# PetropoulakisPanagiotis/ICP-Variants

Measured on AMD Instinct MI355X. Metric: ICP iterations/s (k-NN + point-to-plane linear, 370k-point ETH-Apartment-like pair), higher is better.
Workload: dtype f32

## Files before the change

### icp-variants_amd/csrc/dev_fused.hpp

```cpp
struct RowSlotGen {
    const RowTerms& R;
    static constexpr int N = 27;
    template <int A> __device__ __forceinline__ double get() const { return row_slot<A>(R); }
};
struct P2pGen {
    float s[3], d[3]; double wd;
    static constexpr int N = 22;
    template <int A> __device__ __forceinline__ double get() const {
        double v;
        if constexpr (A < 3) v = (double)s[A];
        else if constexpr (A < 6) v = (double)d[A - 3];
        else if constexpr (A == 6) v = wd;
        else if constexpr (A < 10) v = wd * s[A - 7];
        else if constexpr (A < 13) v = wd * d[A - 10];
        else v = (double)d[(A - 13) / 3] * (wd * s[(A - 13) % 3]);
        return v;
    }
};
#ifndef ICP_FUSED_WAVES
#define ICP_FUSED_WAVES 6
#endif
#ifndef ICP_WAVE_STRIDE
#define ICP_WAVE_STRIDE (ICP_BVH_THREADS > 64 ? 128 : 0)
#endif
#ifndef ICP_DEBUG_WALK_ENDS
#define ICP_DEBUG_WALK_ENDS 0
#endif
#ifndef ICP_DEBUG_TIMES
#define ICP_DEBUG_TIMES 0
#endif
#if ICP_DEBUG_TIMES
#define ICP_STAMP(j) do { if (kp.dbg_steps && lane == 0) kp.dbg_steps[8 * (wave_slot) + (j)] = (int)(unsigned int)wall_clock64(); } while (0)
#define ICP_BUDGET_ROW(slot) ((kp.dbg_steps && 16 * kp.dbg_waves + 8 * 4096 <= kp.n) ? kp.dbg_steps + 8 * kp.dbg_waves + 8 * 4096 + 8 * (slot) : nullptr)
#else
#define ICP_STAMP(j)
#define ICP_BUDGET_ROW(slot) nullptr
#endif

template <int DIM> struct QueryIn {
    float r0, r1, r2;
    float c3, c4, c5;
    float rn0, rn1, rn2;
    int q0;
    float4 st;
    float4 ra, rb;
    float tq[DIM]; int j0;
};
template <int DIM>
__device__ __forceinline__ void fused_front_clear(QueryIn<DIM>& in) {
    in.r0 = 0.f; in.r1 = 0.f; in.r2 = 0.f; in.c3 = 0.f; in.c4 = 0.f; in.c5 = 0.f; in.rn0 = 0.f; in.rn1 = 0.f; in.rn2 = 0.f; in.q0 = -1; in.j0 = -1;
    in.st.x = 0.f; in.st.y = 0.f; in.st.z = 0.f; in.st.w = 0.f; in.ra = in.st; in.rb = in.st;
#pragma unroll
    for (int q = 0; q < DIM; q++) in.tq[q] = 0.f;
}
template <int DIM>
__device__ __forceinline__ void fused_front_loads(const KnnParams& kp, const PostParams& pp, const BvhViewT<DIM>& bv, int k, bool seeded, bool inc, QueryIn<DIM>& in) {
    fused_front_clear<DIM>(in);
    if (k >= 0) {
        const int i = kp.sel ? kp.sel[k] : k;
        in.r0 = kp.sx[i]; in.r1 = kp.sy[i]; in.r2 = kp.sz[i];
        if (DIM == 6) { in.c3 = kp.scr[i]; in.c4 = kp.scg[i]; in.c5 = kp.scb[i]; }
        in.rn0 = pp.snx[i]; in.rn1 = pp.sny[i]; in.rn2 = pp.snz[i];
        in.q0 = seeded ? kp.nn_raw[k] : -1;
        if (inc) in.st = kp.qstate[k];
        if (in.q0 >= 0) {
            if (DIM == 3) { in.ra = *(const float4*)(bv.recs + in.q0); in.rb = *((const float4*)(bv.recs + in.q0) + 1); in.tq[0] = in.ra.x; in.tq[1] = in.ra.y; in.tq[2] = in.ra.z; in.j0 = __float_as_int(in.ra.w); }
            else {
                const BvhLeafT<DIM>* lf = bv.leaves + (in.q0 >> 3);
#pragma unroll
                for (int q = 0; q < DIM; q++) in.tq[q] = lf->c[q][in.q0 & 7];
                in.j0 = lf->idx[in.q0 & 7];
            }
        }
    }
}

__host__ __device__ __forceinline__ int fused_wave_slot(int lb, int w, int mgrid) {
    constexpr int NW = BVH_THREADS / WAVE, S = ICP_WAVE_STRIDE;
    if (S == 0 || NW == 1) return lb * NW + w;
    if (S == 1) return w * mgrid + lb;
    const int g = lb / S, j = lb - g * S;
    return (g + 1) * S <= mgrid ? (g * NW + w) * S + j : lb * NW + w;
}

struct PairOut { bool valid; float s0, s1, s2, d0, d1, d2, n0, n1, n2, wt; };

template <int DIM, bool WIDE, bool XW = false>
__device__ __forceinline__ void fused_search_post(const KnnParams& kp, const BvhViewT<DIM>& bv, const PostParams& pp, int k, bool seeded, bool inc, const float* Pm, const float* Nm,
                                                  QueryIn<DIM>& in, uint2* __restrict__ bvh_lbq, int tid, int wave_slot, PairOut& o) {
    const int lane = tid & 63; (void)lane; (void)wave_slot; (void)seeded;
    o.valid = false; o.s0 = 0.f; o.s1 = 0.f; o.s2 = 0.f; o.d0 = 0.f; o.d1 = 0.f; o.d2 = 0.f; o.n0 = 0.f; o.n1 = 0.f; o.n2 = 0.f; o.wt = 0.f;
    float p[DIM];
#pragma unroll
    for (int q = 0; q < DIM; q++) p[q] = 0.f;
    if (DIM == 6) { p[3 % DIM] = in.c3; p[4 % DIM] = in.c4; p[5 % DIM] = in.c5; }
    float rn0 = in.rn0, rn1 = in.rn1, rn2 = in.rn2;
    float best = FLT_MAX, lb_others = 0.f; int bi = -1, bpos = -1, q0 = in.q0;
    float4 ra = in.ra, rb = in.rb;
#if ICP_DEBUG_TIMES
    float dbg_lbo = 0.f, dbg_lb3 = 0.f, dbg_delta = 0.f; int dbg_l2old = -1; const int dbg_q0old = in.q0;
#endif
    bool need_walk = false, verified = false, two_leaf = false;
    float lb3 = 0.f; int l2 = -1;
    if (k >= 0) {
        float2 st2; st2.x = 0.f; st2.y = __int_as_float(-1);
        xform_point(Pm, in.r0, in.r1, in.r2, p[0], p[1], p[2]);
        if (finite3(p[0], p[1], p[2]) && bv.n_valid > 0) {
            need_walk = true;
            if (q0 >= 0) {
                float d = 0.f;
#pragma unroll
                for (int q = 0; q < DIM; q++) { const float e = p[q] - in.tq[q]; d = (q == 0) ? e * e : d + e * e; }
                if (d < best) { best = d; bi = in.j0; bpos = q0; }
                if (inc && bi >= 0) {
                    const float ex = p[0] - in.st.x, ey = p[1] - in.st.y, ez = p[2] - in.st.z;
                    const float delta = sqrt_up((ex * ex + ey * ey) + ez * ez), sbest = sqrt_up(best);
                    const float lbn = (in.st.w - delta) * 0.999999f;
#if ICP_DEBUG_TIMES
                    dbg_lbo = in.st.w; dbg_lb3 = st2.x; dbg_delta = delta;
#endif
                    if (sbest < lbn) { lb_others = lbn; need_walk = false; verified = true; }
                    else {
                        if (kp.qstate2) st2 = kp.qstate2[k];
#if ICP_DEBUG_TIMES
                        dbg_l2old = __float_as_int(st2.y);
#endif
                        const float lb2 = (st2.x - delta) * 0.999999f;
                        l2 = __float_as_int(st2.y);
                        if (sbest < lb2) { two_leaf = true; lb3 = lb2; }
                    }
                }
            }
        }
    }
    ICP_STAMP(1);
#if ICP_DEBUG_TIMES
    if (kp.dbg_steps && k >= 0 && (need_walk || two_leaf) && seeded) {
        int* r = kp.dbg_steps + 8 * kp.dbg_waves + 8 * (k & 4095);
        r[0] = k; r[1] = __float_as_int(best); r[2] = __float_as_int(dbg_lbo); r[3] = __float_as_int(dbg_lb3); r[4] = __float_as_int(dbg_delta); r[5] = two_leaf ? l2 : -2; r[6] = q0; r[7] = (int)(unsigned int)wall_clock64();
    }
    if (kp.dbg_steps) { const int nw_ = __popcll(__ballot(need_walk && !two_leaf)), nl_ = __popcll(__ballot(two_leaf)); if (lane == 0) { kp.dbg_steps[8 * wave_slot + 6] = nw_ | (nl_ << 8);
            kp.dbg_steps[8 * wave_slot + 7] = (int)((__builtin_amdgcn_s_getreg((31 << 11) | 4) & 0xFFFFu) | (__builtin_amdgcn_s_getreg((31 << 11) | 20) << 16)); } }
#endif
    if (two_leaf) {
        f2 p2[DIM];
#pragma unroll
        for (int q = 0; q < DIM; q++) { p2[q].x = p[q]; p2[q].y = p[q]; }
        float b2 = FLT_MAX, b3 = FLT_MAX; int nl2 = -1;
        const int lf = q0 >> 3;
        if constexpr (DIM == 3) {
#pragma unroll 1
            for (int r = 0; r < 2; r++) {
                const int lx = r ? l2 : lf;
                if (r == 0 || (l2 >= 0 && l2 != lf)) leaf_eval<DIM>(bv.leaves + lx, lx, p2, best, bi, bpos, b2, nl2, b3);
            }
        } else {
            leaf_eval<DIM>(bv.leaves + lf, lf, p2, best, bi, bpos, b2, nl2, b3);
            if (l2 >= 0 && l2 != lf) leaf_eval<DIM>(bv.leaves + l2, l2, p2, best, bi, bpos, b2, nl2, b3);
        }
        lb_others = fminf(sqrt_dn(b2), lb3);
        lb3 = fminf(sqrt_dn(b3), lb3);
        l2 = nl2;
        need_walk = false;
    }
#if ICP_DEBUG_STEPS && !ICP_DEBUG_TIMES
    if (k >= 0 && kp.dbg_steps) kp.dbg_steps[k] = need_walk ? -1 : two_leaf ? -2 : 0;
#endif
#if ICP_DEBUG_TIMES
    if (int* row = ICP_BUDGET_ROW(wave_slot)) { if (lane < 8) row[lane] = 0; }
#endif
    bool walked = false;
    if (__any(need_walk)) {
        walked = true;
        float rn[3] = {rn0, rn1, rn2};
        knn_walk_shared<DIM, BVH_THREADS, typename std::conditional<WIDE, unsigned long long, unsigned int>::type, XW ? 1 : 0>(bv, p, rn, need_walk, best, bi, bpos, lb_others, lb3, l2, bvh_lbq, tid, kp.fault, ICP_BUDGET_ROW(wave_slot));
        rn0 = rn[0]; rn1 = rn[1]; rn2 = rn[2];
        q0 = -2;
        fused_front_clear<DIM>(in);
    }
    ICP_STAMP(2);
#if ICP_DEBUG_TIMES && ICP_DEBUG_WALK_ENDS
    if (k >= 0 && need_walk && seeded) {
        DEV_COUNT(8, 1);
        if (dbg_q0old >= 0 && (bpos >> 3) == (dbg_q0old >> 3)) DEV_COUNT(9, 1);
        if (dbg_l2old >= 0 && (bpos >> 3) == dbg_l2old) DEV_COUNT(10, 1);
    }
#endif
    asm volatile("" : "+v"(k));
    if (k >= 0) {
        if (!verified) knn_store_state<DIM>(kp, k, p, best, bpos, lb_others, lb3, l2);
        else if (kp.d2_out) kp.d2_out[k] = best;
        icp_match_t m;
        if (best <= kp.max_dist) { m.idx = bi; m.weight = 1.f; } else { m.idx = -1; m.weight = 0.f; }
        if (m.idx < 0) { if (pp.matches) pp.matches[k] = m; }
        else {
            if (walked || DIM != 3 || bpos != q0) { ra = *(const float4*)(bv.recs + bpos); rb = *((const float4*)(bv.recs + bpos) + 1); }
            o.d0 = ra.x; o.d1 = ra.y; o.d2 = ra.z; o.n0 = rb.x; o.n1 = rb.y; o.n2 = rb.z;
            o.s0 = p[0]; o.s1 = p[1]; o.s2 = p[2];
            o.valid = post_eval<true>(pp, k, m, o.d0, o.d1, o.d2, o.n0, o.n1, o.n2, __float_as_uint(rb.w), o.s0, o.s1, o.s2, o.wt, rn0, rn1, rn2, Nm);
        }
    }
    ICP_STAMP(3);
}

template <class StoreFn>
__device__ __forceinline__ void fused_block_epilogue(const KnnParams& kp, const PostParams& pp, PairOut& o, uint2* __restrict__ bvh_lbq, int tid, int wave_slot, const StoreFn& store) {
    constexpr int NW = BVH_THREADS / WAVE;
    const int lane = tid & 63, w = tid >> 6; (void)wave_slot; (void)kp;
    __syncthreads();
    double* lds = (double*)bvh_lbq;
    double tot;
    if (!o.valid) { o.s0 = 0.f; o.s1 = 0.f; o.s2 = 0.f; o.d0 = 0.f; o.d1 = 0.f; o.d2 = 0.f; o.n0 = 0.f; o.n1 = 0.f; o.n2 = 0.f; o.wt = 0.f; }
    if (pp.metric == ICP_METRIC_POINT_TO_PLANE) {
        RowTerms R;
        build_rows(0, o.s0, o.s1, o.s2, o.d0, o.d1, o.d2, o.n0, o.n1, o.n2, o.wt, R);
        const RowSlotGen g{R};
        tot = wave_transpose_reduce_gen<6, 0>(g, lane);
    } else {
        const P2pGen g{{o.s0, o.s1, o.s2}, {o.d0, o.d1, o.d2}, (double)o.wt};
        tot = wave_transpose_reduce_gen<6, 0>(g, lane);
    }
    ICP_STAMP(4);
    {
        const unsigned long long vm = __ballot(o.valid);
        const int v = wave_value_of_lane(lane);
        if (v < 32) lds[w * 32 + v] = tot;
        if (lane == 0) lds[NW * 32 + w] = (double)__popcll(vm);
    }
    __syncthreads();
    if (tid < NSUM_USED) {
        double out = 0.0;
        if (tid == SUM_N) { for (int ww = 0; ww < NW; ww++) out += lds[NW * 32 + ww]; }
        else {
            const int v = pp.metric == ICP_METRIC_POINT_TO_PLANE ? tid - SUM_M : tid - 1;
            const int nv = pp.metric == ICP_METRIC_POINT_TO_PLANE ? 27 : 22;
            if (v >= 0 && v < nv) { for (int ww = 0; ww < NW; ww++) out += lds[ww * 32 + v]; }
        }
        store(tid, out);
    }
    ICP_STAMP(5);
}

template <int DIM, bool WIDE, bool MERGED>
__device__ __forceinline__ void fused_matcher_body(const KnnParams& kp, const BvhViewT<DIM>& bv, const int* __restrict__ qorder, const PostParams& pp, const RingParams& rp) {
    extern __shared__ uint2 bvh_lbq[];
    constexpr int NW = BVH_THREADS / WAVE;
    if constexpr (MERGED) { if ((int)blockIdx.x < rp.n_red) { if (BVH_THREADS == RING_THREADS || threadIdx.x < RING_THREADS) ring_reduce_solve(rp); return; } }
    const int n_red = MERGED ? rp.n_red : 0;
    const int mblock = (int)blockIdx.x - n_red, mgrid = (int)gridDim.x - n_red;
    typedef const __attribute__((address_space(4))) float* cfloat_p;
    float Pm[16], Nm[9];
    if constexpr (!MERGED) {
        const cfloat_p pc = (cfloat_p)(const void*)kp.ps->pose; const cfloat_p nc = (cfloat_p)(const void*)kp.ps->nmat;
#pragma unroll
        for (int q = 0; q < 16; q++) Pm[q] = pc[q];
#pragma unroll
        for (int q = 0; q < 9; q++) Nm[q] = nc[q];
    }
    const int tid = threadIdx.x, lane = tid & 63, w = tid >> 6;
    if constexpr (MERGED) { if (rp.st.t0 && blockIdx.x == 0 && tid == 0) *rp.st.t0 = wall_clock64(); }
    const int lb = xcd_contiguous_block(mblock, mgrid);
    const int wave_slot = fused_wave_slot(lb, w, mgrid);
    const int t = wave_slot * BVH_QPW + lane;
    ICP_STAMP(0);
    const int k = ((BVH_QPW == WAVE || lane < BVH_QPW) && t < kp.n) ? (qorder ? qorder[t] : t) : -1;
    const bool seeded = kp.use_prev != 0, inc = kp.incremental && seeded;
    QueryIn<DIM> in;
    fused_front_loads<DIM>(kp, pp, bv, k, seeded, inc, in);
    constexpr bool XW = xw_enabled<DIM, BVH_THREADS>();
    if constexpr (XW) {
        xw_init<BVH_THREADS>(bvh_lbq, tid);
        asm volatile("s_waitcnt lgkmcnt(0)\n\ts_barrier" ::: "memory");
    }
    if constexpr (MERGED) { if (!ring_wait_pose(loop_slot((PoseState*)kp.ps, 0, (int)((blockIdx.x * 2u + (unsigned int)w) % (unsigned int)POSE_REPLICAS)), lane, rp.run_fault, Pm, Nm)) return; }
    PairOut o;
    fused_search_post<DIM, WIDE, XW>(kp, bv, pp, k, seeded, inc, Pm, Nm, in, bvh_lbq, tid, wave_slot, o);
    if constexpr (XW) {
        if (xw_block_is_searching<BVH_THREADS>(bvh_lbq)) {
            constexpr int NT = BVH_THREADS;
            bvh_lbq[3 * NT + tid] = make_uint2(__float_as_uint(o.s0), __float_as_uint(o.s1)); bvh_lbq[4 * NT + tid] = make_uint2(__float_as_uint(o.s2), __float_as_uint(o.d0));
            bvh_lbq[5 * NT + tid] = make_uint2(__float_as_uint(o.d1), __float_as_uint(o.d2)); bvh_lbq[7 * NT + tid] = make_uint2(__float_as_uint(o.n0), __float_as_uint(o.n1));
            bvh_lbq[8 * NT + tid] = make_uint2(__float_as_uint(o.n2), __float_as_uint(o.wt)); bvh_lbq[9 * NT + tid] = make_uint2(o.valid ? 1u : 0u, 0u);
            xw_help<DIM, NT, typename std::conditional<WIDE, unsigned long long, unsigned int>::type>(bv, bvh_lbq, tid, kp.fault, ICP_BUDGET_ROW(wave_slot));
            const uint2 a = bvh_lbq[3 * NT + tid], b = bvh_lbq[4 * NT + tid], c = bvh_lbq[5 * NT + tid], d = bvh_lbq[7 * NT + tid], e = bvh_lbq[8 * NT + tid], f = bvh_lbq[9 * NT + tid];
            o.s0 = __uint_as_float(a.x); o.s1 = __uint_as_float(a.y); o.s2 = __uint_as_float(b.x); o.d0 = __uint_as_float(b.y); o.d1 = __uint_as_float(c.x); o.d2 = __uint_as_float(c.y);
            o.n0 = __uint_as_float(d.x); o.n1 = __uint_as_float(d.y); o.n2 = __uint_as_float(e.x); o.wt = __uint_as_float(e.y); o.valid = f.x != 0u;
        }
    }
    double* partials = pp.partials;
    fused_block_epilogue(kp, pp, o, bvh_lbq, tid, wave_slot, [=](int a, double v) { partials[(size_t)a * mgrid + lb] = v; });
    if constexpr (MERGED) { if (rp.st.block_t1 && tid == 0) rp.st.block_t1[lb] = wall_clock64(); }
}
template <int DIM, bool WIDE>
__global__ __launch_bounds__(BVH_THREADS, DIM == 3 ? ICP_FUSED_WAVES : 4) void k_knn_bvh_post(const KnnParams kp, const BvhViewT<DIM> bv, const int* __restrict__ qorder, const PostParams pp) {
    const RingParams none{};
    fused_matcher_body<DIM, WIDE, false>(kp, bv, qorder, pp, none);
}
template <int DIM, bool WIDE>
__global__ __launch_bounds__(BVH_THREADS, DIM == 3 ? ICP_FUSED_WAVES : 4) void k_knn_bvh_post_ring(const KnnParams kp, const BvhViewT<DIM> bv, const int* __restrict__ qorder, const PostParams pp, const RingParams rp) {
    static_assert(BVH_THREADS >= RING_THREADS, "the reducer blocks are the first RING_THREADS threads of a matcher-sized block");
    fused_matcher_body<DIM, WIDE, true>(kp, bv, qorder, pp, rp);
}
```

### icp-variants_amd/csrc/dev_solve.hpp

```cpp
template <int n, int COPY>
__device__ inline void jacobi_eig_sym(double* A , double* V, double* ev) {
#pragma unroll
    for (int i = 0; i < n; i++) {
#pragma unroll
        for (int j = 0; j < n; j++) V[i * n + j] = (i == j) ? 1.0 : 0.0;
    }
    for (int sweep = 0; sweep < 50; sweep++) {
        double off = 0.0, dg = 0.0;
#pragma unroll
        for (int i = 0; i < n; i++) {
#pragma unroll
            for (int j = 0; j < n; j++) { if (i != j) off += A[i * n + j] * A[i * n + j]; else dg += A[i * n + j] * A[i * n + j]; }
        }
        if (off <= 1e-300 || off <= 1e-34 * dg) break;
#pragma unroll
        for (int p = 0; p < n - 1; p++) {
#pragma unroll
            for (int q = p + 1; q < n; q++) {
                const double apq = A[p * n + q];
                if (apq != 0.0) {
                    const double theta = (A[q * n + q] - A[p * n + p]) / (2.0 * apq);
                    const double t = (theta >= 0 ? 1.0 : -1.0) / (fabs(theta) + sqrt(theta * theta + 1.0));
                    const double c = 1.0 / sqrt(t * t + 1.0), s = t * c;
#pragma unroll
// ... 266 lines not shown
}
template <int COPY = 0>
__device__ __forceinline__ bool solve_p2plane_lanes(const SolveParams& sp, const double* tot ) {
    if (!(sp.update_pose && sp.metric == ICP_METRIC_POINT_TO_PLANE && sp.phase == 0 && tot[SUM_N] > 0)) return false;
    PoseState* ps = sp.ps;
    const float* npose = p2plane_lanes_core<COPY>(tot + SUM_M, ps->pose);
    if (!npose) return false;
    const int tid = threadIdx.x;
    if (tid == 0 && sp.sums_out) for (int a = 0; a < NSUM; a++) sp.sums_out[a] = tot[a];
    if (tid >= 64 && tid < 70) {
        const int k = tid - 64; const double n = tot[SUM_N];
        if (k < 3) ps->mean_s[k] = (float)(tot[SUM_S + k] / n); else ps->mean_d[k - 3] = (float)(tot[SUM_D + k - 3] / n);
    }
    if (tid < 16) { ps->pose[tid] = npose[tid]; if (sp.stats) sp.stats->pose[tid] = npose[tid]; }
    if (tid >= 32 && tid < 41) ps->nmat[tid - 32] = normal_matrix_entry(npose, tid - 32);
    if (tid == 33 && sp.stats) {
        sp.stats->n_src = sp.n_src; sp.stats->n_valid = (int)tot[SUM_N];
        sp.stats->rmse = -1.f; sp.stats->benchmark_error = -1.f; sp.stats->status = ICP_OK;
    }
    return true;
}

template <bool WITH_SYMMETRIC, int COPY = 0>
__device__ inline void solve_generic(const SolveParams& sp, const double* tot) {
    if (sp.sums_out) for (int a = 0; a < NSUM; a++) sp.sums_out[a] = tot[a];
    PoseState* ps = sp.ps;
    const double n = tot[SUM_N];
    if (sp.phase == 0) {
        float ms[3] = {0, 0, 0}, md[3] = {0, 0, 0};
        if (n > 0) for (int k = 0; k < 3; k++) { ms[k] = (float)(tot[SUM_S + k] / n); md[k] = (float)(tot[SUM_D + k] / n); }
        for (int k = 0; k < 3; k++) { ps->mean_s[k] = ms[k]; ps->mean_d[k] = md[k]; }
    }
    if (!sp.update_pose) return;
    if (sp.metric == ICP_METRIC_SYMMETRIC && sp.phase == 0) return;
    int status = ICP_OK;
    float dT[16];
    for (int i = 0; i < 16; i++) dT[i] = (i % 5 == 0) ? 1.f : 0.f;
    if (!(n > 0)) {
        status = ICP_ERR_NO_CORRESPONDENCES;
    } else if (sp.metric == ICP_METRIC_POINT_TO_PLANE) {
        double x[6];
        solve_normal_svd<COPY>(tot + SUM_M, x);
        const float al = (float)x[0], be = (float)x[1], ga = (float)x[2];
        const float ca = (float)cos((double)al), sa = (float)sin((double)al);
        const float cb = (float)cos((double)be), sb = (float)sin((double)be);
        const float cg = (float)cos((double)ga), sg = (float)sin((double)ga);
        const float Rx[9] = {1, 0, 0, 0, ca, -sa, 0, sa, ca}, Ry[9] = {cb, 0, sb, 0, 1, 0, -sb, 0, cb}, Rz[9] = {cg, -sg, 0, sg, cg, 0, 0, 0, 1};
        float Rxy[9], R[9];
        mat3_mul_f32(Rx, Ry, Rxy); mat3_mul_f32(Rxy, Rz, R);
        const float t[3] = {(float)x[3], (float)x[4], (float)x[5]};
        set_pose_f32(dT, R, t);
    } else if (sp.metric == ICP_METRIC_POINT_TO_POINT) {
        const double* m = tot + SUM_M;
        const float msf[3] = {ps->mean_s[0], ps->mean_s[1], ps->mean_s[2]}, mdf[3] = {ps->mean_d[0], ps->mean_d[1], ps->mean_d[2]};
        __shared__ double A[9], Rd[9];
        for (int j = 0; j < 3; j++) for (int k = 0; k < 3; k++)
            A[j * 3 + k] = m[7 + j * 3 + k] - m[4 + j] * (double)msf[k] - (double)mdf[j] * m[1 + k] + m[0] * (double)mdf[j] * (double)msf[k];
        double mom = 0.0;
        for (int i = 0; i < 9; i++) mom = fmax(mom, fabs(m[7 + i]));
        float R[9];
        procrustes_rotation<COPY>(A, (RANK_CUT3 * RANK_CUT3) * mom, Rd);
        for (int i = 0; i < 9; i++) R[i] = (float)Rd[i];
        const float tr[3] = {mdf[0] - msf[0], mdf[1] - msf[1], mdf[2] - msf[2]};
        float t[3];
        for (int r = 0; r < 3; r++) {
            const float Rt = R[r * 3] * tr[0] + (R[r * 3 + 1] * tr[1] + R[r * 3 + 2] * tr[2]);
            const float Rm = R[r * 3] * mdf[0] + (R[r * 3 + 1] * mdf[1] + R[r * 3 + 2] * mdf[2]);
            t[r] = (Rt - Rm) + mdf[r];
        }
        set_pose_f32(dT, R, t);
    } else if constexpr (WITH_SYMMETRIC) {
        __shared__ double M[36], g[6], x[6], ywork[6];
        __shared__ int colp[6];
        int q = 0;
        for (int a = 0; a < 6; a++) for (int c = a; c < 6; c++) { M[a * 6 + c] = tot[SUM_M + q]; M[c * 6 + a] = tot[SUM_M + q]; q++; }
        for (int a = 0; a < 6; a++) g[a] = tot[SUM_M + 21 + a];
        const float lambda = 0.0001f; const float l2 = lambda * lambda;
        for (int a = 0; a < 6; a++) M[a * 6 + a] += (double)l2;
        solve_fullpiv_lu6<COPY>(M, g, x, colp, ywork);
        const float at[3] = {(float)x[0], (float)x[1], (float)x[2]}, tt[3] = {(float)x[3], (float)x[4], (float)x[5]};
        const float tan_theta = sqrtf(at[0] * at[0] + (at[1] * at[1] + at[2] * at[2]));
        const float ax[3] = {at[0] / tan_theta, at[1] / tan_theta, at[2] / tan_theta};
        const float sin_theta = (float)((double)tan_theta / sqrt(1.0 + (double)(tan_theta * tan_theta)));
        const float cos_theta = sin_theta / tan_theta;
        const float t[3] = {tt[0] * cos_theta, tt[1] * cos_theta, tt[2] * cos_theta};
        const float K[9] = {0, -ax[2], ax[1], ax[2], 0, -ax[0], -ax[1], ax[0], 0};
        float Ks[9], KK[9], Rod[9];
        const float omc = 1 - cos_theta;
        for (int i = 0; i < 9; i++) Ks[i] = omc * K[i];
        mat3_mul_f32(Ks, K, KK);
        for (int i = 0; i < 9; i++) Rod[i] = ((i % 4 == 0) ? 1.f : 0.f) + (sin_theta * K[i] + KK[i]);
        const float I3[9] = {1, 0, 0, 0, 1, 0, 0, 0, 1}, zero[3] = {0, 0, 0};
        const float md[3] = {ps->mean_d[0], ps->mean_d[1], ps->mean_d[2]}, nms[3] = {-ps->mean_s[0], -ps->mean_s[1], -ps->mean_s[2]};
        float Tm[16], Tt[16], Ts[16], Rm[16], t1[16], t2[16];
        set_pose_f32(Tm, I3, md); set_pose_f32(Tt, I3, t); set_pose_f32(Ts, I3, nms); set_pose_f32(Rm, Rod, zero);
        mat4_mul_f32(Tm, Rm, t1); mat4_mul_f32(t1, Tt, t2); mat4_mul_f32(t2, Rm, t1); mat4_mul_f32(t1, Ts, dT);
    }
    if (status == ICP_OK) {
        float np[16];
        mat4_mul_f32(dT, ps->pose, np);
        for (int i = 0; i < 16; i++) ps->pose[i] = np[i];
        normal_matrix_from_pose(ps->pose, ps->nmat);
    }
    if (sp.stats) {
        sp.stats->n_src = sp.n_src;
        sp.stats->n_valid = (int)n;
        for (int i = 0; i < 16; i++) sp.stats->pose[i] = ps->pose[i];
        sp.stats->rmse = -1.f;
        sp.stats->benchmark_error = -1.f;
        sp.stats->status = status;
    }
}

template <bool WITH_SYMMETRIC = true, int COPY = 0>
__device__ __forceinline__ void solve_tail(const SolveParams& sp, const double* tot) {
    if (solve_p2plane_lanes<COPY>(sp, tot)) return;
    if (threadIdx.x == 0) solve_generic<WITH_SYMMETRIC, COPY>(sp, tot);
}

constexpr int SOLVE_THREADS = 256;
constexpr unsigned long long TOTAL_SENTINEL = 0xFFF8D1CEC0DE5EEDull;
constexpr int SPIN_LIMIT = 1 << 22;
constexpr int SOLVE_INFLIGHT = 12;
__global__ __launch_bounds__(SOLVE_THREADS) void k_reduce_solve(const SolveParams sp) {
#include "dev_body_reduce_solve.hpp"
}


#ifndef ICP_POSE_REPLICAS
#define ICP_POSE_REPLICAS 16
#endif
constexpr int POSE_REPLICAS = ICP_POSE_REPLICAS;
constexpr size_t POSE_REPLICA_STRIDE = 4096 + 128;
__device__ __host__ __forceinline__ PoseState* loop_slot(PoseState* base, int g, int replica) {
    return (PoseState*)((char*)base + ((size_t)g * POSE_REPLICAS + (size_t)replica) * POSE_REPLICA_STRIDE);
}
__global__ void k_run_init(const PoseState src, PoseState* ps_copy, PoseState* slots, int n_slots, unsigned long long* totals, int n_totals, int* zero_words, int n_zero,
                           unsigned long long* stamps, int n_stamps) {
    const int t = blockIdx.x * blockDim.x + threadIdx.x;
    const int n_slot_granules = n_slots * POSE_REPLICAS * 16;
    if (t < n_slot_granules) {
        const int g = t / (POSE_REPLICAS * 16), r = (t / 16) % POSE_REPLICAS, q = t & 15;
        unsigned long long* dst = (unsigned long long*)loop_slot(slots, g, r) + q;
        *dst = g == 0 ? ((const unsigned long long*)&src)[q] : ~0ull;
        if (g == 0 && r == 0 && ps_copy) ((unsigned long long*)ps_copy)[q] = ((const unsigned long long*)&src)[q];
    } else if (t < n_slot_granules + n_totals) totals[t - n_slot_granules] = ~0ull;
    else if (t < n_slot_granules + n_totals + n_zero) zero_words[t - n_slot_granules - n_totals] = 0;
    else if (t < n_slot_granules + n_totals + n_zero + n_stamps) stamps[t - n_slot_granules - n_totals - n_zero] = 0ull;
}
constexpr unsigned long long GRANULE_EMPTY = ~0ull;
#ifndef ICP_RING_SLEEP
#define ICP_RING_SLEEP 4
#endif
struct RingStamps {
    unsigned long long* t0; unsigned long long* block_t1;
    const unsigned long long* prev_block_t1; unsigned long long* prev_t1;
    unsigned long long* end;
};
struct RingParams {
    const double* red_partials; int red_nblocks;
    unsigned long long* totals_row;
    const PoseState* ps_in;
    PoseState* ps_out;
    icp_iter_stats* stats; int n_src;
    PoseState* final_out;
    int* words_out;
    int* run_fault;
    int n_red;
    ConvergeParams cv;
    RingStamps st;
};
__device__ __forceinline__ unsigned long long granule_of(unsigned int lo, unsigned int hi) {
    const unsigned long long g = ((unsigned long long)hi << 32) | lo;
    return g == GRANULE_EMPTY ? g ^ 1ull : g;
}
constexpr int RING_THREADS = 128;
#ifndef ICP_DEBUG_TIMES
#define ICP_DEBUG_TIMES 0
#endif
#if ICP_DEBUG_TIMES
__device__ int g_ring_dbg[(NSUM_USED + 1) * 8];
#define RING_STAMP(a, j) do { if (threadIdx.x == 0 && !rp.final_out) g_ring_dbg[8 * (a) + (j)] = (int)(unsigned int)wall_clock64(); } while (0)
#else
#define RING_STAMP(a, j)
#endif
__device__ __forceinline__ void ring_close(const RingParams& rp) {
    if (threadIdx.x != 0) return;
    if (rp.words_out) {
        int wds[16];
#pragma unroll
        for (int k = 0; k < 16; k++) wds[k] = __hip_atomic_load(rp.run_fault + k, __ATOMIC_RELAXED, __HIP_MEMORY_SCOPE_AGENT);
#pragma unroll
        for (int k = 0; k < 16; k++) rp.words_out[k] = wds[k];
    }
    if (rp.st.end) *rp.st.end = wall_clock64();
}
__device__ __forceinline__ void ring_reduce_solve(const RingParams& rp) {
    __shared__ double tot[NSUM];
    __shared__ double wsum[4];
    __shared__ unsigned int slot_words[32];
    __shared__ int give_up;
    const int tid = threadIdx.x, lane = tid & 63, w = tid >> 6, a = blockIdx.x;
    RING_STAMP(a, 0);
    if (a == 0 && tid == 0 && rp.st.t0) *rp.st.t0 = wall_clock64();
    if (a == 0 && rp.ps_in->fault) {
        { const unsigned int* src = (const unsigned int*)rp.ps_in; for (int q = tid; q < 16 * POSE_REPLICAS; q += RING_THREADS) __hip_atomic_store((unsigned long long*)loop_slot(rp.ps_out, 0, q >> 4) + (q & 15), granule_of(src[2 * (q & 15)], src[2 * (q & 15) + 1]), __ATOMIC_RELAXED, __HIP_MEMORY_SCOPE_AGENT);
          if (rp.final_out && tid < 32) ((unsigned int*)rp.final_out)[tid] = src[tid]; }
        ring_close(rp);
        return;
    }
    {
        const double* __restrict__ row = rp.red_partials + (size_t)a * rp.red_nblocks;
        double x0 = 0.0, x1 = 0.0;
        for (int b0 = 0; b0 < rp.red_nblocks; b0 += SOLVE_INFLIGHT * SOLVE_THREADS) {
            double v0[SOLVE_INFLIGHT], v1[SOLVE_INFLIGHT];
#pragma unroll
            for (int j = 0; j < SOLVE_INFLIGHT; j++) {
                const int b = b0 + j * SOLVE_THREADS + tid;
                v0[j] = b < rp.red_nblocks ? row[b] : 0.0;
                v1[j] = b + RING_THREADS < rp.red_nblocks ? row[b + RING_THREADS] : 0.0;
            }
#pragma unroll
            for (int j = 0; j < SOLVE_INFLIGHT; j++) {
                const int b = b0 + j * SOLVE_THREADS + tid;
                if (b < rp.red_nblocks) x0 += v0[j];
                if (b + RING_THREADS < rp.red_nblocks) x1 += v1[j];
            }
        }
        for (int off = 32; off > 0; off >>= 1) { x0 += __shfl_down(x0, off, WAVE); x1 += __shfl_down(x1, off, WAVE); }
        if (lane == 0) { wsum[w] = x0; wsum[2 + w] = x1; }
    }
    RING_STAMP(a, 1);
    __syncthreads();
    if (tid == 0) {
        double x = wsum[0];
        for (int k = 1; k < 4; k++) x += wsum[k];
        const unsigned long long bits = (unsigned long long)__double_as_longlong(x);
        __hip_atomic_store(rp.totals_row + a, granule_of((unsigned int)bits, (unsigned int)(bits >> 32)), __ATOMIC_RELAXED, __HIP_MEMORY_SCOPE_AGENT);
    }
    RING_STAMP(a, 2);
    if (a == 1 && rp.st.prev_t1) {
        static_assert(RING_THREADS == 2 * WAVE, "two wave maxima meet below");
        __shared__ unsigned long long tmax[RING_THREADS / WAVE];
        unsigned long long m = 0ull;
        for (int b = tid; b < rp.red_nblocks; b += RING_THREADS) { const unsigned long long v = rp.st.prev_block_t1[b]; m = v > m ? v : m; }
        for (int off = 32; off > 0; off >>= 1) { const unsigned long long v = __shfl_down(m, off, WAVE); m = v > m ? v : m; }
        if (lane == 0) tmax[w] = m;
        __syncthreads();
        if (tid == 0) *rp.st.prev_t1 = tmax[0] > tmax[1] ? tmax[0] : tmax[1];
    }
    if (a != 0) return;
    if (tid == 0) give_up = 0;
    __syncthreads();
    if (tid < NSUM) {
        double v = 0.0;
        if (tid < NSUM_USED) {
            unsigned long long bits = GRANULE_EMPTY;
            for (int spin = 0; spin < SPIN_LIMIT; spin++) {
                bits = __hip_atomic_load(rp.totals_row + tid, __ATOMIC_RELAXED, __HIP_MEMORY_SCOPE_AGENT);
                if (bits != GRANULE_EMPTY) break;
                __builtin_amdgcn_s_sleep(2);
            }
            if (bits == GRANULE_EMPTY) give_up = 1;
            v = __longlong_as_double((long long)bits);
        }
        tot[tid] = v;
    }
    __syncthreads();
    RING_STAMP(NSUM_USED, 0);
    const PoseState* pin = rp.ps_in;
    const double n = tot[SUM_N];
    int fault = 0, status = ICP_OK;
    const float* npose = nullptr;
    if (give_up) { fault = 1; if (tid == 0) atomicOr(rp.run_fault, 1); }
    else if (n > 0) { npose = p2plane_lanes_core(tot + SUM_M, pin->pose); if (!npose) fault = 2; }
    else status = ICP_ERR_NO_CORRESPONDENCES;
    RING_STAMP(NSUM_USED, 1);
    int code = fault;
    if (rp.cv.on && !fault) {
        if (tid < WAVE && converge_step(rp.cv, npose ? npose : pin->pose, pin->pose, status == ICP_OK, tid)) code = SLOT_STOPPED;
    }
    if (tid < 16) slot_words[tid] = __float_as_uint(npose ? npose[tid] : pin->pose[tid]);
    if (tid >= 32 && tid < 41) slot_words[16 + tid - 32] = __float_as_uint(npose ? normal_matrix_entry(npose, tid - 32) : pin->nmat[tid - 32]);
    if (tid >= 64 && tid < 70) {
        const int k = tid - 64;
        slot_words[25 + k] = __float_as_uint(n > 0 ? (float)(tot[(k < 3 ? SUM_S : SUM_D - 3) + k] / n) : 0.f);
    }
    if (tid == 0) slot_words[31] = (unsigned int)code;
    __syncthreads();
    for (int q = tid; q < 16 * POSE_REPLICAS; q += RING_THREADS)
        __hip_atomic_store((unsigned long long*)loop_slot(rp.ps_out, 0, q >> 4) + (q & 15), granule_of(slot_words[2 * (q & 15)], slot_words[2 * (q & 15) + 1]), __ATOMIC_RELAXED, __HIP_MEMORY_SCOPE_AGENT);
    RING_STAMP(NSUM_USED, 2);
    if (rp.final_out && tid < 32) ((unsigned int*)rp.final_out)[tid] = slot_words[tid];
    if (rp.stats && !fault) {
        if (tid < 16) rp.stats->pose[tid] = __uint_as_float(slot_words[tid]);
        if (tid == 16) { rp.stats->n_src = rp.n_src; rp.stats->n_valid = (int)n; rp.stats->rmse = -1.f; rp.stats->benchmark_error = -1.f; rp.stats->status = status; }
    }
    ring_close(rp);
}
__global__ __launch_bounds__(RING_THREADS) void k_ring_reduce_solve(const RingParams rp) { ring_reduce_solve(rp); }

__device__ __forceinline__ bool ring_wait_pose(const PoseState* slot, int lane, int* run_fault, float (&Pm)[16], float (&Nm)[9]) {
    const unsigned long long* g = (const unsigned long long*)slot;
    unsigned long long v = 0ull;
    bool ok = false;
    for (int spin = 0; spin < SPIN_LIMIT; spin++) {
        if (lane < 16) v = __hip_atomic_load(g + lane, __ATOMIC_RELAXED, __HIP_MEMORY_SCOPE_AGENT);
        if (!__any(lane < 16 && v == GRANULE_EMPTY)) { ok = true; break; }
        __builtin_amdgcn_s_sleep(ICP_RING_SLEEP);
    }
    if (!ok) { if (lane == 0) atomicOr(run_fault, 1); return false; }
    const int lo = (int)(unsigned int)v, hi = (int)(unsigned int)(v >> 32);
#pragma unroll
    for (int q = 0; q < 16; q++) Pm[q] = __int_as_float(__builtin_amdgcn_readlane((q & 1) ? hi : lo, q >> 1));
#pragma unroll
    for (int q = 0; q < 9; q++) Nm[q] = __int_as_float(__builtin_amdgcn_readlane(((16 + q) & 1) ? hi : lo, (16 + q) >> 1));
    return __builtin_amdgcn_readlane(hi, 15) == 0;
}
```

### icp-variants_amd/csrc/host_launch.hpp

```cpp
namespace {
struct MergeLaunch { RingParams rp; const PoseState* slot; double* partials; };

constexpr size_t WALK_LDS_BYTES = (size_t)ICP_SHARE_ROWS * BVH_THREADS * 8;
template <int DIM> size_t fused_lds_bytes() {
    const size_t red_bytes = (size_t)(BVH_THREADS / WAVE) * 33 * 8;
    return (WALK_LDS_BYTES > red_bytes ? WALK_LDS_BYTES : red_bytes) + xw_lds_bytes<DIM, BVH_THREADS>();
}
int post_nblocks(int n) { const int nb = (n + POST_THREADS - 1) / POST_THREADS; return nb > POST_BLOCKS ? POST_BLOCKS : nb < 1 ? 1 : nb; }
template <class K> K pick_wide(int Lq, K narrow, K wide) { return Lq <= 8 ? narrow : wide; }

struct QuerySet { const Cloud* cl; const int* sel; int n; int pretransformed; bool use_colors; bool seed_prev; const int* order; bool keep_records = false; };

int ensure_qpack(icp_ctx* c, int n) {
    if ((size_t)n <= c->q_cap && c->qpack.p) return ICP_OK;
    int rc;
    c->q_cap = ((size_t)n + 63) / 64 * 64;
    if ((rc = ensure(c, c->qpack, c->q_cap * 28))) return rc;
    set_view(c->nn_raw, c->qpack.p, c->q_cap * 4); set_view(c->qstate, c->qpack.as<char>() + c->q_cap * 4, c->q_cap * 16);
    set_view(c->qstate2, c->qpack.as<char>() + c->q_cap * 20, c->q_cap * 8);
    return ICP_OK;
}

KnnParams knn_params(const icp_ctx* c, const Cloud& q, const int* sel, int n) {
    KnnParams kp; memset(&kp, 0, sizeof(kp));
    kp.sx = q.x.as<float>(); kp.sy = q.y.as<float>(); kp.sz = q.z.as<float>(); kp.scr = q.cr.as<float>(); kp.scg = q.cg.as<float>(); kp.scb = q.cb.as<float>();
    kp.sel = sel; kp.n = n;
    kp.tx = c->tgt.x.as<float>(); kp.ty = c->tgt.y.as<float>(); kp.tz = c->tgt.z.as<float>();
    kp.tcr = c->tgt.cr.as<float>(); kp.tcg = c->tgt.cg.as<float>(); kp.tcb = c->tgt.cb.as<float>();
    kp.mpad = c->tgt.npad; kp.max_dist = c->prm.max_distance; kp.nseg = 1;
    return kp;
}

PostParams make_post_params(icp_ctx* c, const Cloud& src, const int* sel, int n) {
    const icp_params& p = c->prm;
    PostParams pp;
    pp.sx = src.x.as<float>(); pp.sy = src.y.as<float>(); pp.sz = src.z.as<float>();
    pp.snx = src.nx.as<float>(); pp.sny = src.ny.as<float>(); pp.snz = src.nz.as<float>();
    pp.srgba = src.rgba.as<uint32_t>(); pp.sel = sel; pp.n = n;
    pp.tx = c->tgt.x.as<float>(); pp.ty = c->tgt.y.as<float>(); pp.tz = c->tgt.z.as<float>();
    pp.tnx = c->tgt.nx.as<float>(); pp.tny = c->tgt.ny.as<float>(); pp.tnz = c->tgt.nz.as<float>(); pp.trgba = c->tgt.rgba.as<uint32_t>();
    pp.ps = c->ps.as<PoseState>(); pp.matches = c->matches.as<icp_match_t>();
    pp.metric = p.metric; pp.weighting = p.weighting; pp.rejection = p.rejection;
    pp.max_dist = p.max_distance; pp.cos_reject = c->cos_reject; pp.partials = c->partials.as<double>();
    return pp;
}

template <int DIM>
int launch_bvh_query(icp_ctx* c, Bvh& b, const CoordPtrs<DIM>& cp, const KnnParams& kp, const int* order, int n, const Cloud* fuse, bool keep_records, int* fused_blocks, const MergeLaunch* ml = nullptr) {
    int rc;
    if (!b.valid && (rc = build_bvh<DIM>(c, b, cp))) return rc;
    const BvhViewT<DIM> bv = make_view<DIM>(b, cp);
    const int nb = fuse ? fused_nblocks(n) : (n + BVH_THREADS - 1) / BVH_THREADS;
    if (fuse) {
        if ((rc = ensure(c, c->partials, (size_t)(nb > POST_BLOCKS ? nb : POST_BLOCKS) * NSUM * 8))) return rc;
        PostParams pp = make_post_params(c, *fuse, kp.sel, n);
        KnnParams kf = kp; kf.out = nullptr;
        if (!keep_records) { pp.matches = nullptr; kf.d2_out = nullptr; }
        const size_t lds = fused_lds_bytes<DIM>();
        if (ml) {
            kf.ps = ml->slot; pp.ps = ml->slot; pp.partials = ml->partials; kf.fault = ml->rp.run_fault;
            const auto ring = pick_wide(b.Lq, k_knn_bvh_post_ring<DIM, false>, k_knn_bvh_post_ring<DIM, true>);
            hipLaunchKernelGGL(ring, dim3(nb + ml->rp.n_red), dim3(BVH_THREADS), lds, c->stream, kf, bv, order, pp, ml->rp);
        }
        else hipLaunchKernelGGL(pick_wide(b.Lq, k_knn_bvh_post<DIM, false>, k_knn_bvh_post<DIM, true>), dim3(nb), dim3(BVH_THREADS), lds, c->stream, kf, bv, order, pp);
        *fused_blocks = nb;
    } else hipLaunchKernelGGL(k_knn_bvh<DIM>, dim3(nb), dim3(BVH_THREADS), WALK_LDS_BYTES, c->stream, kp, bv, order);
    HIPCK(c, hipGetLastError());
    return ICP_OK;
}

int launch_match(icp_ctx* c, const QuerySet& q, int* fused_blocks = nullptr, const MergeLaunch* ml = nullptr) {
    const icp_params& p = c->prm;
    int rc;
    if (fused_blocks) *fused_blocks = 0;
    if ((rc = ensure(c, c->matches, (size_t)q.n * sizeof(icp_match_t))) || (rc = ensure(c, c->d2, (size_t)q.n * 4))) return rc;
    if (p.matching == ICP_MATCH_PROJECTIVE) {
        ProjParams pp;
        pp.sx = q.cl->x.as<float>(); pp.sy = q.cl->y.as<float>(); pp.sz = q.cl->z.as<float>(); pp.sel = q.sel; pp.n = q.n;
        pp.tx = c->tgt.x.as<float>(); pp.ty = c->tgt.y.as<float>(); pp.tz = c->tgt.z.as<float>();
        pp.width = p.width; pp.height = p.height; pp.fx = p.fx; pp.fy = p.fy; pp.mx = p.cx; pp.my = p.cy; pp.window = 12;
        pp.ps = c->ps.as<PoseState>(); pp.pretransformed = q.pretransformed; pp.max_dist = p.max_distance;
        pp.out = c->matches.as<icp_match_t>(); pp.d2_out = c->d2.as<float>();
        hipLaunchKernelGGL(k_projective, dim3((q.n + 255) / 256), dim3(256), 0, c->stream, pp);
        HIPCK(c, hipGetLastError());
        return ICP_OK;
    }
    KnnParams kp = knn_params(c, *q.cl, q.sel, q.n);
    kp.ps = c->ps.as<PoseState>(); kp.pretransformed = q.pretransformed; kp.fault = &c->ps.as<PoseState>()->fault;
    kp.out = c->matches.as<icp_match_t>(); kp.d2_out = c->d2.as<float>();
    if (p.knn_backend == ICP_KNN_LBVH) {
        if ((rc = ensure_qpack(c, q.n))) return rc;
        kp.nn_raw = c->nn_raw.as<int>(); kp.use_prev = q.seed_prev ? 1 : 0;
#if ICP_DEBUG_STEPS
        if ((rc = ensure(c, c->dbg_steps, (size_t)q.n * 4))) return rc;
        kp.dbg_steps = c->dbg_steps.as<int>(); kp.dbg_waves = fused_nblocks(q.n) * (BVH_THREADS / WAVE);
#endif
        if (p.knn_incremental && !q.pretransformed) {
            kp.qstate = c->qstate.as<float4>(); kp.qstate2 = c->qstate2.as<float2>(); kp.incremental = 1;
        }
        const Cloud* fuse = (fused_blocks != nullptr && p.metric != ICP_METRIC_SYMMETRIC && p.metric != ICP_METRIC_GICP && p.metric != ICP_METRIC_COLORED && !q.pretransformed) ? q.cl : nullptr;
        if (q.use_colors) return launch_bvh_query<6>(c, c->bvh6, target_coords6(c), kp, q.order, q.n, fuse, q.keep_records, fused_blocks, fuse ? ml : nullptr);
        return launch_bvh_query<3>(c, c->bvh, target_coords3(c), kp, q.order, q.n, fuse, q.keep_records, fused_blocks, fuse ? ml : nullptr);
    }
    const int bx = (q.n + WAVE - 1) / WAVE;
    const int nch = kp.mpad / KNN_CH;
    int nseg = 1;
    if (bx < 1024) { nseg = (2048 + bx - 1) / bx; if (nseg > nch / 4) nseg = nch / 4; if (nseg < 1) nseg = 1; }
    kp.nseg = nseg;
    if (nseg > 1) {
        if ((rc = ensure(c, c->best64, (size_t)q.n * 8))) return rc;
        kp.best64 = c->best64.as<unsigned long long>();
        const unsigned long long init = ((unsigned long long)0x7F7FFFFFu << 32) | 0xFFFFFFFFull;
        hipLaunchKernelGGL(k_fill_u64, dim3((q.n + 255) / 256), dim3(256), 0, c->stream, kp.best64, q.n, init);
    }
    if (q.use_colors) hipLaunchKernelGGL(k_knn_brute<6>, dim3(bx, nseg), dim3(256), 0, c->stream, kp);
    else              hipLaunchKernelGGL(k_knn_brute<3>, dim3(bx, nseg), dim3(256), 0, c->stream, kp);
    if (nseg > 1)
        hipLaunchKernelGGL(k_knn_finalize, dim3((q.n + 255) / 256), dim3(256), 0, c->stream, kp.best64, q.n, p.max_distance,
                           c->matches.as<icp_match_t>(), c->d2.as<float>());
    HIPCK(c, hipGetLastError());
    return ICP_OK;
}

int rearm_handover(icp_ctx* c) {
    int rc;
    if ((rc = ensure(c, c->totals, NSUM * 8 + 8))) return rc;
    HIPCK(c, hipMemsetAsync(c->totals.p, 0, NSUM * 8 + 8, c->stream));
    hipLaunchKernelGGL(k_fill_u64, dim3(1), dim3(64), 0, c->stream, c->totals.as<unsigned long long>(), NSUM, TOTAL_SENTINEL);
    HIPCK(c, hipGetLastError());
    return ICP_OK;
}

const int* level_src_orig(icp_ctx* c, const Cloud& src) {
    if (&src == &c->src) return nullptr;
    for (auto& kv : c->levels) if (&kv.second.sorted == &src) return kv.second.sorted_idx.as<int>();
    for (auto& kv : c->nss_held) if (&kv.second.lv.sorted == &src) return kv.second.lv.sorted_idx.as<int>();
    return nullptr;
}

GicpPost gicp_post_params(icp_ctx* c, const Cloud& src) {
    GicpPost g; memset(&g, 0, sizeof(g));
    const bool own_t = c->gicp_opt.covariance_k == 0, own_s = own_t;
    g.tnx = own_t ? c->tgt.nx.as<float>() : c->gicp_n[0][0].as<float>(); g.tny = own_t ? c->tgt.ny.as<float>() : c->gicp_n[0][1].as<float>(); g.tnz = own_t ? c->tgt.nz.as<float>() : c->gicp_n[0][2].as<float>();
    g.snx = own_s ? c->src.nx.as<float>() : c->gicp_n[1][0].as<float>(); g.sny = own_s ? c->src.ny.as<float>() : c->gicp_n[1][1].as<float>(); g.snz = own_s ? c->src.nz.as<float>() : c->gicp_n[1][2].as<float>();
    g.src_orig = level_src_orig(c, src);
    g.one_minus_eps = 1.0 - (double)c->gicp_opt.epsilon;
    return g;
}

ColoredPost colored_post_params(icp_ctx* c) {
    ColoredPost g;
    g.gx = c->col_grad[0].as<float>(); g.gy = c->col_grad[1].as<float>(); g.gz = c->col_grad[2].as<float>();
    g.lambda = (double)c->col_opt.lambda_geometric;
    return g;
}

bool robust_on(const icp_ctx* c) { return c->rob_opt.kernel != ICP_ROBUST_NONE || c->rob_opt.overlap < 1.f; }

int robust_prepare(icp_ctx* c, int slots) {
// ... 166 lines not shown
```

Baseline: 35790.

## Poll the ring pose once per block via LDS and defer front loads past the wait

```diff
diff --git a/icp-variants_amd/csrc/dev_fused.hpp b/icp-variants_amd/csrc/dev_fused.hpp
--- a/icp-variants_amd/csrc/dev_fused.hpp
+++ b/icp-variants_amd/csrc/dev_fused.hpp
@@ -37,35 +37,47 @@
 #define ICP_BUDGET_ROW(slot) nullptr
 #endif
 
-template <int DIM> struct QueryIn {
+typedef float float4v __attribute__((ext_vector_type(4)));
+template <int DIM, bool DEFER = false> struct QueryIn {
+    typedef typename std::conditional<DEFER, float4v, float4>::type V4;
     float r0, r1, r2;
     float c3, c4, c5;
     float rn0, rn1, rn2;
     int q0;
-    float4 st;
-    float4 ra, rb;
+    V4 st;
+    V4 ra, rb;
     float tq[DIM]; int j0;
 };
-template <int DIM>
-__device__ __forceinline__ void fused_front_clear(QueryIn<DIM>& in) {
+template <int DIM, bool DEFER = false>
+__device__ __forceinline__ void fused_front_clear(QueryIn<DIM, DEFER>& in) {
     in.r0 = 0.f; in.r1 = 0.f; in.r2 = 0.f; in.c3 = 0.f; in.c4 = 0.f; in.c5 = 0.f; in.rn0 = 0.f; in.rn1 = 0.f; in.rn2 = 0.f; in.q0 = -1; in.j0 = -1;
     in.st.x = 0.f; in.st.y = 0.f; in.st.z = 0.f; in.st.w = 0.f; in.ra = in.st; in.rb = in.st;
 #pragma unroll
     for (int q = 0; q < DIM; q++) in.tq[q] = 0.f;
 }
-template <int DIM>
-__device__ __forceinline__ void fused_front_loads(const KnnParams& kp, const PostParams& pp, const BvhViewT<DIM>& bv, int k, bool seeded, bool inc, QueryIn<DIM>& in) {
-    fused_front_clear<DIM>(in);
+template <int DIM, bool DEFER = false>
+__device__ __forceinline__ void fused_front_loads(const KnnParams& kp, const PostParams& pp, const BvhViewT<DIM>& bv, int k, bool seeded, bool inc, QueryIn<DIM, DEFER>& in) {
+    typedef typename QueryIn<DIM, DEFER>::V4 V4;
+    if constexpr (DEFER) {
+        in.r0 = 0.f; in.r1 = 0.f; in.r2 = 0.f; in.c3 = 0.f; in.c4 = 0.f; in.c5 = 0.f; in.rn0 = 0.f; in.rn1 = 0.f; in.rn2 = 0.f; in.q0 = -1;
+        if constexpr (DIM != 3) {
+            in.j0 = -1;
+#pragma unroll
+            for (int q = 0; q < DIM; q++) in.tq[q] = 0.f;
+        }
+    } else fused_front_clear<DIM, DEFER>(in);
     if (k >= 0) {
         const int i = kp.sel ? kp.sel[k] : k;
         in.r0 = kp.sx[i]; in.r1 = kp.sy[i]; in.r2 = kp.sz[i];
         if (DIM == 6) { in.c3 = kp.scr[i]; in.c4 = kp.scg[i]; in.c5 = kp.scb[i]; }
         in.rn0 = pp.snx[i]; in.rn1 = pp.sny[i]; in.rn2 = pp.snz[i];
         in.q0 = seeded ? kp.nn_raw[k] : -1;
-        if (inc) in.st = kp.qstate[k];
+        if (inc) in.st = *(const V4*)(kp.qstate + k);
         if (in.q0 >= 0) {
-            if (DIM == 3) { in.ra = *(const float4*)(bv.recs + in.q0); in.rb = *((const float4*)(bv.recs + in.q0) + 1); in.tq[0] = in.ra.x; in.tq[1] = in.ra.y; in.tq[2] = in.ra.z; in.j0 = __float_as_int(in.ra.w); }
-            else {
+            if (DIM == 3) {
+                in.ra = *(const V4*)(bv.recs + in.q0); in.rb = *((const V4*)(bv.recs + in.q0) + 1);
+                if constexpr (!DEFER) { in.tq[0] = in.ra.x; in.tq[1] = in.ra.y; in.tq[2] = in.ra.z; in.j0 = __float_as_int(in.ra.w); }
+            } else {
                 const BvhLeafT<DIM>* lf = bv.leaves + (in.q0 >> 3);
 #pragma unroll
                 for (int q = 0; q < DIM; q++) in.tq[q] = lf->c[q][in.q0 & 7];
@@ -73,6 +85,18 @@
             }
         }
     }
+}
+
+template <int DIM>
+__device__ __forceinline__ void fused_front_arrive(QueryIn<DIM, true>& in) {
+    asm volatile("" : "+v"(in.st));
+    if constexpr (DIM == 3) asm volatile("" : "+v"(in.ra), "+v"(in.rb));
+}
+
+template <int DIM> constexpr size_t fused_pose_lds_offset() {
+    static_assert((size_t)ICP_SHARE_ROWS * BVH_THREADS * 8 >= (size_t)(BVH_THREADS / WAVE) * 33 * 8, "the block reduction fits in the walk's rows");
+    static_assert(xw_lds_bytes<DIM, BVH_THREADS>() % 8 == 0, "the pose copy is read in 8-byte granules");
+    return (size_t)ICP_SHARE_ROWS * BVH_THREADS * 8 + xw_lds_bytes<DIM, BVH_THREADS>();
 }
 
 __host__ __device__ __forceinline__ int fused_wave_slot(int lb, int w, int mgrid) {
@@ -85,9 +109,9 @@
 
 struct PairOut { bool valid; float s0, s1, s2, d0, d1, d2, n0, n1, n2, wt; };
 
-template <int DIM, bool WIDE, bool XW = false>
+template <int DIM, bool WIDE, bool XW = false, bool DEFER = false>
 __device__ __forceinline__ void fused_search_post(const KnnParams& kp, const BvhViewT<DIM>& bv, const PostParams& pp, int k, bool seeded, bool inc, const float* Pm, const float* Nm,
-                                                  QueryIn<DIM>& in, uint2* __restrict__ bvh_lbq, int tid, int wave_slot, PairOut& o) {
+                                                  QueryIn<DIM, DEFER>& in, uint2* __restrict__ bvh_lbq, int tid, int wave_slot, PairOut& o) {
     const int lane = tid & 63; (void)lane; (void)wave_slot; (void)seeded;
     o.valid = false; o.s0 = 0.f; o.s1 = 0.f; o.s2 = 0.f; o.d0 = 0.f; o.d1 = 0.f; o.d2 = 0.f; o.n0 = 0.f; o.n1 = 0.f; o.n2 = 0.f; o.wt = 0.f;
     float p[DIM];
@@ -96,7 +120,8 @@
     if (DIM == 6) { p[3 % DIM] = in.c3; p[4 % DIM] = in.c4; p[5 % DIM] = in.c5; }
     float rn0 = in.rn0, rn1 = in.rn1, rn2 = in.rn2;
     float best = FLT_MAX, lb_others = 0.f; int bi = -1, bpos = -1, q0 = in.q0;
-    float4 ra = in.ra, rb = in.rb;
+    float4 ra, rb;
+    ra.x = in.ra.x; ra.y = in.ra.y; ra.z = in.ra.z; ra.w = in.ra.w; rb.x = in.rb.x; rb.y = in.rb.y; rb.z = in.rb.z; rb.w = in.rb.w;
 #if ICP_DEBUG_TIMES
     float dbg_lbo = 0.f, dbg_lb3 = 0.f, dbg_delta = 0.f; int dbg_l2old = -1; const int dbg_q0old = in.q0;
 #endif
@@ -109,9 +134,11 @@
             need_walk = true;
             if (q0 >= 0) {
                 float d = 0.f;
-#pragma unroll
-                for (int q = 0; q < DIM; q++) { const float e = p[q] - in.tq[q]; d = (q == 0) ? e * e : d + e * e; }
-                if (d < best) { best = d; bi = in.j0; bpos = q0; }
+                constexpr bool FROM_RA = DEFER && DIM == 3;
+                const float tq3[3] = {in.ra.x, in.ra.y, in.ra.z};
+#pragma unroll
+                for (int q = 0; q < DIM; q++) { const float e = p[q] - (FROM_RA ? tq3[q % 3] : in.tq[q]); d = (q == 0) ? e * e : d + e * e; }
+                if (d < best) { best = d; bi = FROM_RA ? __float_as_int(in.ra.w) : in.j0; bpos = q0; }
                 if (inc && bi >= 0) {
                     const float ex = p[0] - in.st.x, ey = p[1] - in.st.y, ez = p[2] - in.st.z;
                     const float delta = sqrt_up((ex * ex + ey * ey) + ez * ez), sbest = sqrt_up(best);
@@ -176,7 +203,7 @@
         knn_walk_shared<DIM, BVH_THREADS, typename std::conditional<WIDE, unsigned long long, unsigned int>::type, XW ? 1 : 0>(bv, p, rn, need_walk, best, bi, bpos, lb_others, lb3, l2, bvh_lbq, tid, kp.fault, ICP_BUDGET_ROW(wave_slot));
         rn0 = rn[0]; rn1 = rn[1]; rn2 = rn[2];
         q0 = -2;
-        fused_front_clear<DIM>(in);
+        fused_front_clear<DIM, DEFER>(in);
     }
     ICP_STAMP(2);
 #if ICP_DEBUG_TIMES && ICP_DEBUG_WALK_ENDS
@@ -265,16 +292,25 @@
     ICP_STAMP(0);
     const int k = ((BVH_QPW == WAVE || lane < BVH_QPW) && t < kp.n) ? (qorder ? qorder[t] : t) : -1;
     const bool seeded = kp.use_prev != 0, inc = kp.incremental && seeded;
-    QueryIn<DIM> in;
-    fused_front_loads<DIM>(kp, pp, bv, k, seeded, inc, in);
+    QueryIn<DIM, MERGED> in;
     constexpr bool XW = xw_enabled<DIM, BVH_THREADS>();
-    if constexpr (XW) {
-        xw_init<BVH_THREADS>(bvh_lbq, tid);
+    if constexpr (MERGED) {
+        unsigned long long* const pose_lds = (unsigned long long*)((char*)bvh_lbq + fused_pose_lds_offset<DIM>());
+        if constexpr (XW) xw_init<BVH_THREADS>(bvh_lbq, tid);
+        ring_pose_lds_init(pose_lds, tid);
         asm volatile("s_waitcnt lgkmcnt(0)\n\ts_barrier" ::: "memory");
-    }
-    if constexpr (MERGED) { if (!ring_wait_pose(loop_slot((PoseState*)kp.ps, 0, (int)((blockIdx.x * 2u + (unsigned int)w) % (unsigned int)POSE_REPLICAS)), lane, rp.run_fault, Pm, Nm)) return; }
+        fused_front_loads<DIM, true>(kp, pp, bv, k, seeded, inc, in);
+        if (!ring_wait_pose_lds(loop_slot((PoseState*)kp.ps, 0, (int)((blockIdx.x * 2u + (unsigned int)w) % (unsigned int)POSE_REPLICAS)), pose_lds, lane, rp.run_fault, Pm, Nm)) return;
+        fused_front_arrive<DIM>(in);
+    } else {
+        fused_front_loads<DIM, false>(kp, pp, bv, k, seeded, inc, in);
+        if constexpr (XW) {
+            xw_init<BVH_THREADS>(bvh_lbq, tid);
+            asm volatile("s_waitcnt lgkmcnt(0)\n\ts_barrier" ::: "memory");
+        }
+    }
     PairOut o;
-    fused_search_post<DIM, WIDE, XW>(kp, bv, pp, k, seeded, inc, Pm, Nm, in, bvh_lbq, tid, wave_slot, o);
+    fused_search_post<DIM, WIDE, XW, MERGED>(kp, bv, pp, k, seeded, inc, Pm, Nm, in, bvh_lbq, tid, wave_slot, o);
     if constexpr (XW) {
         if (xw_block_is_searching<BVH_THREADS>(bvh_lbq)) {
             constexpr int NT = BVH_THREADS;
diff --git a/icp-variants_amd/csrc/dev_solve.hpp b/icp-variants_amd/csrc/dev_solve.hpp
--- a/icp-variants_amd/csrc/dev_solve.hpp
+++ b/icp-variants_amd/csrc/dev_solve.hpp
@@ -442,6 +442,9 @@
 #ifndef ICP_RING_SLEEP
 #define ICP_RING_SLEEP 4
 #endif
+#ifndef ICP_RING_LDS_SLEEP
+#define ICP_RING_LDS_SLEEP 2
+#endif
 struct RingStamps {
     unsigned long long* t0; unsigned long long* block_t1;
     const unsigned long long* prev_block_t1; unsigned long long* prev_t1;
@@ -590,14 +593,31 @@
 }
 __global__ __launch_bounds__(RING_THREADS) void k_ring_reduce_solve(const RingParams rp) { ring_reduce_solve(rp); }
 
-__device__ __forceinline__ bool ring_wait_pose(const PoseState* slot, int lane, int* run_fault, float (&Pm)[16], float (&Nm)[9]) {
-    const unsigned long long* g = (const unsigned long long*)slot;
+constexpr int RING_POSE_LDS_BYTES = 16 * 8 + 16;
+__device__ __forceinline__ void ring_pose_lds_init(unsigned long long* pl, int tid) {
+    if (tid < 16) pl[tid] = GRANULE_EMPTY;
+    if (tid == 16) *(int*)(pl + 16) = 0;
+}
+__device__ __forceinline__ bool ring_wait_pose_lds(const PoseState* slot, unsigned long long* pl, int lane, int* run_fault, float (&Pm)[16], float (&Nm)[9]) {
     unsigned long long v = 0ull;
     bool ok = false;
-    for (int spin = 0; spin < SPIN_LIMIT; spin++) {
-        if (lane < 16) v = __hip_atomic_load(g + lane, __ATOMIC_RELAXED, __HIP_MEMORY_SCOPE_AGENT);
-        if (!__any(lane < 16 && v == GRANULE_EMPTY)) { ok = true; break; }
-        __builtin_amdgcn_s_sleep(ICP_RING_SLEEP);
+    int first = 0;
+    if (lane == 0) first = __hip_atomic_fetch_add((int*)(pl + 16), 1, __ATOMIC_RELAXED, __HIP_MEMORY_SCOPE_WORKGROUP) == 0;
+    if (__builtin_amdgcn_readfirstlane(first)) {
+        const unsigned long long* g = (const unsigned long long*)slot;
+        for (int spin = 0; spin < SPIN_LIMIT; spin++) {
+            if (lane < 16) v = __hip_atomic_load(g + lane, __ATOMIC_RELAXED, __HIP_MEMORY_SCOPE_AGENT);
+            if (!__any(lane < 16 && v == GRANULE_EMPTY)) { ok = true; break; }
+            __builtin_amdgcn_s_sleep(ICP_RING_SLEEP);
+        }
+        if (!ok) v = lane == 15 ? 1ull << 32 : 0ull;
+        if (lane < 16) __hip_atomic_store(pl + lane, v, __ATOMIC_RELAXED, __HIP_MEMORY_SCOPE_WORKGROUP);
+    } else {
+        for (int spin = 0; spin < SPIN_LIMIT; spin++) {
+            if (lane < 16) v = __hip_atomic_load(pl + lane, __ATOMIC_RELAXED, __HIP_MEMORY_SCOPE_WORKGROUP);
+            if (!__any(lane < 16 && v == GRANULE_EMPTY)) { ok = true; break; }
+            __builtin_amdgcn_s_sleep(ICP_RING_LDS_SLEEP);
+        }
     }
     if (!ok) { if (lane == 0) atomicOr(run_fault, 1); return false; }
     const int lo = (int)(unsigned int)v, hi = (int)(unsigned int)(v >> 32);
diff --git a/icp-variants_amd/csrc/host_launch.hpp b/icp-variants_amd/csrc/host_launch.hpp
--- a/icp-variants_amd/csrc/host_launch.hpp
+++ b/icp-variants_amd/csrc/host_launch.hpp
@@ -3,8 +3,7 @@
 
 constexpr size_t WALK_LDS_BYTES = (size_t)ICP_SHARE_ROWS * BVH_THREADS * 8;
 template <int DIM> size_t fused_lds_bytes() {
-    const size_t red_bytes = (size_t)(BVH_THREADS / WAVE) * 33 * 8;
-    return (WALK_LDS_BYTES > red_bytes ? WALK_LDS_BYTES : red_bytes) + xw_lds_bytes<DIM, BVH_THREADS>();
+    return fused_pose_lds_offset<DIM>() + RING_POSE_LDS_BYTES;
 }
 int post_nblocks(int n) { const int nb = (n + POST_THREADS - 1) / POST_THREADS; return nb > POST_BLOCKS ? POST_BLOCKS : nb < 1 ? 1 : nb; }
 template <class K> K pick_wide(int Lq, K narrow, K wide) { return Lq <= 8 ? narrow : wide; }
```

After: 36070, median of 4. No clear change (+0.8%).
